# facebookresearch/robust_cvd

Hardware: NVIDIA H100
Metric: flow_residual_constraints_per_sec_per_gn_iteration (higher is better)
Workload: dtype f64

## Files before the change

robust_cvd_b200/csrc/rcvd_api.cu:

```cuda
#include <algorithm>
#include <chrono>
#include <cmath>
#include <cstdarg>
#include <cstdio>
#include <cstring>
#include <dlfcn.h>
#include <limits>
#include <map>
#include <mutex>
#include <string>
#include <vector>

#include <cub/device/device_segmented_sort.cuh>
#include "rcvd_eval.cuh"
#include "rcvd_linalg.cuh"
#include "rcvd_update.cuh"
#include "rcvd_plan.h"
#include "rcvd_cg.cuh"
#include "rcvd_selinv.cuh"
#include "rcvd_host.h"

using namespace rcvd;

static thread_local std::string g_err = "";
// ... 107 lines not shown
  if (e >= nf * nf) return;
  const int i = e / nf, j = e % nf;
  const HBlock hbk = hb[b];
  if (hbk.r == hbk.c && j > i) return;
  const double v = H[(size_t)b * npad * npad + (size_t)i * npad + j];
  const size_t U = (size_t)N * nf;
  const int ur = uperm[hbk.r], uc = uperm[hbk.c];
  out[((size_t)ur * nf + i) * U + (size_t)uc * nf + j] = v;
  out[((size_t)uc * nf + j) * U + (size_t)ur * nf + i] = v;
}

enum { LP_POTRF_SMEM = 0, LP_POTRF_PANEL, LP_TRSM_LL4, LP_TRSM_LL2, LP_TRSM_GEMM, LP_UPD_TMA1, LP_UPD_TMA2, LP_SUB_LEVEL, LP_SUB_FUSED,
       LP_TRINV, LP_OTHER, LP_UPD_TMA1_MULTI, LP_TRSM_STREAMED, LP_N };

struct RecordSet {
  const int width, nframes;
  std::vector<int32_t> frames; std::vector<int64_t> offsets{0}; std::vector<float> records;
  RecordTiles dev = {}; int num_tiles = 0;
  const float* caller_records = nullptr;
  RecordSet(int width_, int nframes_) : width(width_), nframes(nframes_) {}
  int groups() const { return (int)offsets.size() - 1; }
  int64_t count() const { return offsets.back(); }
};

struct rcvd_problem {
  rcvd_config cfg; Layout L; int N = 0; int device = 0;
  cudaStream_t stream = nullptr;
  std::vector<uint8_t> in_range; std::vector<double> median, adaptive;
  RecordSet pairs{6, 2}, trips{10, 1}, dpairs{6, 2};
  std::vector<int32_t> struct_pairs;
  int first_frame = 0, last_frame = -1;
  int32_t* d_blk_of = nullptr; uint8_t *d_in_range = nullptr, *d_active = nullptr;
  double *d_median = nullptr, *d_adaptive = nullptr; float* d_scale_locs = nullptr; int nscale = 0;
  double *d_x = nullptr, *d_xc = nullptr, *d_xsave = nullptr;
  double *d_g = nullptr, *d_S = nullptr, *d_diagH = nullptr, *d_lmdiag = nullptr, *d_D2 = nullptr, *d_gs = nullptr, *d_rhs = nullptr, *d_ytmp = nullptr,
         *d_y = nullptr, *d_Sy = nullptr, *d_Hy = nullptr, *d_partial = nullptr, *d_scal = nullptr;
  double* h_scal = nullptr;
  int part_reg = 0, part_trip = 0, part_dp = 0, npartial = 0;
  double *d_H = nullptr, *d_Lb = nullptr, *d_T = nullptr, *d_invL = nullptr, *d_invT = nullptr;
  HBlock *d_hblocks = nullptr, *d_lblocks = nullptr; int* d_fail = nullptr;
  int* d_potrf_progress = nullptr;
  FactorKernels fk = {};
  FactorPlan plan;
  int *d_lvl_frames = nullptr; TrsmTask* d_trsm_tasks = nullptr; int2* d_upd_pairs = nullptr; SolveTask* d_fwd_tasks = nullptr;
  SubTask* d_sub_tasks = nullptr; int* d_sub_counters = nullptr; int* d_sub_need = nullptr;
  cudaGraphExec_t solve_graph = nullptr;
  bool structure_ready = false;
  int nranks = 1, rank = 0; nccl::Comm comm = nullptr;
  int64_t launches = 0, graph_launches = 0;
  std::vector<double> h_state; bool state_dirty = true; bool overlap = true; int order_slack = 4;
  cudaStream_t side_stream = nullptr; cudaEvent_t ev_fork = nullptr, ev_join = nullptr;
  std::vector<cudaEvent_t> ev_side;
  cudaStream_t inv_stream = nullptr; cudaEvent_t ev_inv_join = nullptr;
  double *d_g2 = nullptr, *d_delta = nullptr; int* h_fail = nullptr;
  cudaEvent_t ev[8] = {nullptr};
  std::vector<void*> allocs;
  std::vector<std::pair<int, cudaEvent_t>>* prof = nullptr;
  bool eval_only = false;
  bool records_sorted = false;
  int fast_path = 1;
  bool dist_enabled = true, graph_warm = false, force_full_H = false;
  int *d_lvl_own = nullptr, *d_load_lblocks = nullptr, *d_own_hblocks = nullptr, *d_uperm = nullptr;
  UpdItem* d_upd_items = nullptr; CUtensorMap tmapT; int num_sms = 0, upd_ipc = 0, upd_order = 1;
  std::vector<double> level_ms;
  bool factored = false;
  int64_t paths[LP_N] = {0}, graph_paths[LP_N] = {0};
  bool use_cg = false; int64_t factor_budget = -1; uint64_t total_mem = 0;
  LinearStorage storage = {}; int64_t linear_bytes = 0;
  double cg_eta = kCgEta;
  double *d_cg_r = nullptr, *d_cg_z = nullptr, *d_cg_p = nullptr, *d_cg_q = nullptr, *d_cg_slots = nullptr, *d_cg_part = nullptr;
  int *d_cg_frames = nullptr, *d_cg_off = nullptr, *d_cg_ids = nullptr; CgState* d_cg = nullptr;
  int64_t cg_iterations = 0; int cg_max = 0, cg_capped = 0, cg_steps = 0, cg_last = 0;
  bool sel_ready = false; SelPlan sel;
  SelTile* d_sel_tiles = nullptr; SelOp* d_sel_ops = nullptr; SelTrmm* d_sel_trmm = nullptr; int *d_sel_row_off = nullptr, *d_sel_row_blk = nullptr;
  int64_t sel_launches[5] = {0}; double sel_ms[3] = {0.0, 0.0, 0.0};
  rcvd_problem() {}
};

template <class... Params, class... Args>
static int launch(rcvd_problem* p, void (*kernel)(Params...), dim3 grid, dim3 block, size_t smem, cudaStream_t s, bool pdl, Args... args) {
  if (int rc = launch_kernel(kernel, grid, block, smem, s, pdl, args...)) return rc;
  p->launches += 1;
  return RCVD_OK;
}

template <class T> static int dalloc(rcvd_problem* p, T** ptr, size_t count) {
  *ptr = nullptr;
  if (count == 0) count = 1;
  cudaError_t e = cudaMallocAsync((void**)ptr, count * sizeof(T), p->stream);
  if (e != cudaSuccess) return set_err(RCVD_ERR_CUDA, "cudaMallocAsync(%zu bytes) failed: %s", count * sizeof(T), cudaGetErrorString(e));
  p->allocs.push_back(*ptr);
  return RCVD_OK;
}
template <class T> static int upload(rcvd_problem* p, T** ptr, const std::vector<T>& v) {
  int rc = dalloc(p, ptr, v.size()); if (rc) return rc;
  if (!v.empty()) CK(cudaMemcpyAsync(*ptr, v.data(), v.size() * sizeof(T), cudaMemcpyHostToDevice, p->stream));
  return RCVD_OK;
}
template <class T> static std::vector<T> frames_to_internal(const std::vector<int>& uperm, const T* src, size_t src_stride, size_t dst_stride, size_t count, T pad = T()) {
  std::vector<T> out(uperm.size() * dst_stride, pad);
  for (size_t i = 0; i < uperm.size(); ++i) std::copy_n(src + (size_t)uperm[i] * src_stride, count, out.begin() + i * dst_stride);
  return out;
}
template <class T> static void frames_to_caller(const std::vector<int>& uperm, const T* src, size_t src_stride, T* dst, size_t dst_stride, size_t count) {
  for (size_t i = 0; i < uperm.size(); ++i) std::copy_n(src + i * src_stride, count, dst + (size_t)uperm[i] * dst_stride);
}
// ... 200 lines not shown
  if (fk.trsm_ll4) {
    CK(cudaFuncSetAttribute(k_trsm_ll<4>, cudaFuncAttributeMaxDynamicSharedMemorySize, (int)fk.trsm_ll4_bytes));
    CK(cudaFuncSetAttribute(k_trsm_ll<4, true>, cudaFuncAttributeMaxDynamicSharedMemorySize, (int)fk.trsm_ll4_bytes));
  }
  if (fk.potrf_smem) CK(cudaFuncSetAttribute(k_potrf_smem, cudaFuncAttributeMaxDynamicSharedMemorySize, (int)fk.potrf_bytes));
  return RCVD_OK;
}

static int build_structure(rcvd_problem* p) {
  if (p->nranks > 1 && !p->dpairs.frames.empty()) return set_err(RCVD_ERR_INVALID, "depth-normalisation pairs are not sharded: they need a single-GPU problem (nranks = 1)");
  free_all(p);
  CK(cudaSetDevice(p->device));
  std::vector<int32_t> graph = p->struct_pairs.empty() ? p->pairs.frames : p->struct_pairs;
  graph.insert(graph.end(), p->dpairs.frames.begin(), p->dpairs.frames.end());
  if (const char* e = make_factor_plan(p->plan, p->cfg, graph, p->trips.frames, p->order_slack, p->nranks, p->rank, p->dist_enabled, p->num_sms))
    return set_err(RCVD_ERR_INVALID, "%s", e);
  p->storage = linear_storage(p->plan, p->N, p->L.npad);
  p->use_cg = p->nranks == 1 && !p->eval_only && p->storage.cholesky > (p->factor_budget >= 0 ? p->factor_budget : cholesky_budget(p->total_mem));
  while (p->ev_side.size() < 2 * p->plan.levels.size()) { cudaEvent_t e; CK(cudaEventCreateWithFlags(&e, cudaEventDisableTiming)); p->ev_side.push_back(e); }
  int rc;
  if ((rc = upload_plan(p)) || (rc = set_up_problem_data(p)) || (rc = allocate_storage(p))) return rc;
  CK(cudaStreamSynchronize(p->stream));
  p->structure_ready = true;
  return RCVD_OK;
}

static int allreduce(rcvd_problem* p, double* buf, size_t count) {
  if (p->nranks <= 1) return RCVD_OK;
  const int r = nccl::AllReduce(buf, buf, count, nccl::kFloat64, nccl::kSum, p->comm, p->stream);
  if (r != 0) return set_err(RCVD_ERR_NCCL, "ncclAllReduce failed: %s", nccl::GetErrorString ? nccl::GetErrorString(r) : "?");
  return RCVD_OK;
}
struct Seg { size_t first, count; };
static int grouped(rcvd_problem* p, double* base, size_t unit, const std::vector<Seg>& segs, bool bcast) {
  int r = nccl::GroupStart();
  for (size_t i = 0; i < segs.size() && r == 0; ++i) {
    if (segs[i].count == 0) continue;
    const int root = (int)(i % (size_t)p->nranks);
    double* ptr = base + segs[i].first * unit;
    r = bcast ? nccl::Broadcast(ptr, ptr, segs[i].count * unit, nccl::kFloat64, root, p->comm, p->stream)
              : nccl::Reduce(ptr, ptr, segs[i].count * unit, nccl::kFloat64, nccl::kSum, root, p->comm, p->stream);
  }
  const int r2 = nccl::GroupEnd();
  if (r == 0) r = r2;
  if (r != 0) return set_err(RCVD_ERR_NCCL, "grouped NCCL %s failed: %s", bcast ? "broadcast" : "reduce", nccl::GetErrorString ? nccl::GetErrorString(r) : "?");
  return RCVD_OK;
}

struct FactorSolve {
  enum { P_LOAD = 0, P_POTRF, P_TRINV, P_TRSM, P_GEMM, P_SOLVE };
  rcvd_problem* p; const FactorPlan& pl; const FactorKernels& fk; const int N, npad, strips; cudaStream_t st, side, inv;
  int prof_level = 0;
  bool side_used = false, inv_used = false;
  int side_joined = -1;

  explicit FactorSolve(rcvd_problem* p_)
      : p(p_), pl(p_->plan), fk(p_->fk), N(p_->N), npad(p_->L.npad), strips((npad + kTrsmStrip - 1) / kTrsmStrip), st(p_->stream), side(p_->side_stream),
        inv(p_->inv_stream) {}

  void mark(int cls) {
    if (!p->prof) return;
    cudaEvent_t e; cudaEventCreate(&e); cudaEventRecord(e, st); p->prof->push_back({cls < 0 ? cls : (cls | (prof_level << 8)), e});
  }
  template <class... Params, class... Args>
  int launch(int path, void (*kernel)(Params...), dim3 grid, dim3 block, size_t smem, cudaStream_t s, bool pdl, Args... args) {
    if (int rc = ::launch(p, kernel, grid, block, smem, s, pdl, args...)) return rc;
    p->paths[path]++;
    return RCVD_OK;
  }
  int wait(cudaStream_t waiter, cudaStream_t from, cudaEvent_t e) {
    CK(cudaEventRecord(e, from)); CK(cudaStreamWaitEvent(waiter, e, 0));
    return RCVD_OK;
  }
  int join_all(int level) {
    if (side_used) { if (int rc = wait(st, side, p->ev_join)) return rc; side_joined = 2 * level - 1; }
    if (inv_used) { if (int rc = wait(st, inv, p->ev_inv_join)) return rc; inv_used = false; }
    return RCVD_OK;
  }

  bool trsm_deep(const Level& v) const { return strips * v.ntrsm <= p->num_sms && fk.trsm_ll4; }
  bool streamed(const Level& v) const {
    return fk.trsm_ll && v.nown > 0 && v.ntrsm > 0 && fk.potrf_smem && strips * v.ntrsm <= (trsm_deep(v) ? 1 : fk.trsm2_ctas_per_sm) * p->num_sms;
  }

  int factor_diagonal(const int* frames, int nfr, bool pdl) {
    if (fk.potrf_smem)
      return launch(LP_POTRF_SMEM, k_potrf_smem, dim3(nfr), dim3(kPotrfSmemThreads), fk.potrf_bytes, st, pdl, p->d_Lb, p->d_invT, frames, npad,
                    p->d_fail, p->d_potrf_progress);
    for (int jb = 0; jb < npad / 16; ++jb) {
      if (int rc = launch(LP_POTRF_PANEL, k_potrf_panel, dim3(nfr), dim3(kPotrfThreads), 0, st, false, p->d_Lb, p->d_invT, frames, npad, jb, p->d_fail)) return rc;
      const int m = npad - (jb + 1) * 16, n64 = (m + 63) / 64;
      if (m > 0) { if (int rc = launch(LP_OTHER, k_potrf_trail, dim3(n64 * (n64 + 1) / 2, nfr), dim3(128), 0, st, false, p->d_Lb, frames, npad, jb)) return rc; }
    }
    return RCVD_OK;
  }

  int trsm(const Level& lv, const int* frames, int nfr, bool chain) {
    const bool inv_stream = fk.trsm_ll && p->overlap;
    if (inv_stream) { if (int rc = wait(inv, st, p->ev_fork)) return rc; inv_used = true; }
    if (int rc = launch(LP_TRINV, k_trinv, dim3(npad / 16, nfr), dim3(256), fk.trinv_bytes, inv_stream ? inv : st, false,
                        p->d_Lb, p->d_invT, p->d_invL, frames, npad)) return rc;
    mark(P_TRINV);
    if (lv.ntrsm == 0) return RCVD_OK;
    int rc;
    if (fk.trsm_ll) {
      const bool deep = trsm_deep(lv);
      decltype(&k_trsm_ll<2>) kernel = deep ? (chain ? k_trsm_ll<4, true> : k_trsm_ll<4>) : (chain ? k_trsm_ll<2, true> : k_trsm_ll<2>);
      if (chain) p->paths[LP_TRSM_STREAMED]++;
      rc = launch(deep ? LP_TRSM_LL4 : LP_TRSM_LL2, kernel, dim3(strips, lv.ntrsm), dim3(128), deep ? fk.trsm_ll4_bytes : fk.trsm_ll2_bytes, st, chain,
                  p->d_T, p->d_Lb, p->d_invT, p->d_trsm_tasks + lv.trsm_off, npad, chain ? p->d_potrf_progress : nullptr);
    } else {
      const int tiles = (npad + 63) / 64;
      rc = launch(LP_TRSM_GEMM, k_gemm_nt, dim3(tiles, tiles, lv.ntrsm), dim3(128), 0, st, false, p->d_T, p->d_Lb, p->d_invL,
                  p->d_trsm_tasks + lv.trsm_off, npad);
    }
    if (rc) return rc;
    mark(P_TRSM);
    return RCVD_OK;
  }

  int update(cudaStream_t s, int off, int n) {
    const UpdItem* items = p->d_upd_items + (size_t)p->upd_order * pl.upd_items.size() + off;
    if (n <= p->num_sms)
      return launch(LP_UPD_TMA2, k_update_tma<2>, dim3(n), dim3(UpdShape<2>::threads), upd_smem_bytes(pl.upd_rb, 2), s, false,
                    p->tmapT, p->d_Lb, items, n, p->d_upd_pairs, npad, pl.upd_neff, pl.upd_rb, 0);
    int grid = upd_ctas(n, p->num_sms);
    if (p->upd_ipc > 0) grid = std::max(grid, (n + p->upd_ipc - 1) / p->upd_ipc);
    if (grid < n) p->paths[LP_UPD_TMA1_MULTI]++;
    return launch(LP_UPD_TMA1, k_update_tma<1>, dim3(grid), dim3(UpdShape<1>::threads), upd_smem_bytes(pl.upd_rb, 1), s, false,
                  p->tmapT, p->d_Lb, items, n, p->d_upd_pairs, npad, pl.upd_neff, pl.upd_rb, 0);
  }

  int updates(int li) {
    const Level& lv = pl.levels[li];
    const bool u2 = lv.nit2[0] + lv.nit2[1] > 0;
    const bool fork_late = li + 1 < (int)pl.levels.size() && streamed(pl.levels[li + 1]);
    if (p->overlap && u2 && !fork_late) { if (int rc = wait(side, st, p->ev_fork)) return rc; }
    if (p->overlap) {
      int s = -1;
      for (int q = side_joined + 1; q < 2 * li; ++q) { const Level& v = pl.levels[q / 2]; if (v.nit2[q % 2] > 0 && v.join[q % 2] <= li) s = q; }
      if (s >= 0) { CK(cudaStreamWaitEvent(st, p->ev_side[s], 0)); side_joined = s; }
    }
    if (lv.nit > 0) { if (int rc = update(st, lv.it_off, lv.nit)) return rc; mark(P_GEMM); }
    if (p->overlap && u2 && fork_late) { if (int rc = wait(side, st, p->ev_fork)) return rc; }
    for (int h = 0; h < 2; ++h) if (lv.nit2[h] > 0) {
      if (int rc = update(p->overlap ? side : st, lv.it2_off[h], lv.nit2[h])) return rc;
      mark(P_GEMM);
      if (p->overlap) { CK(cudaEventRecord(p->ev_side[2 * li + h], side)); side_used = true; }
    }
    return RCVD_OK;
  }

  int broadcast_level(int li) {
    std::vector<Seg> segs;
    for (int q = 0; q < p->nranks; ++q) segs.push_back({(size_t)pl.tseg[(li * p->nranks + q) * 2], (size_t)pl.tseg[(li * p->nranks + q) * 2 + 1]});
    return grouped(p, p->d_T, (size_t)npad * npad, segs, true);
  }
  int phase_boundary() {
    if (int rc = join_all(pl.LB)) return rc;
    const size_t bsz = (size_t)npad * npad;
    std::vector<Seg> invs, tr;
    for (int q = 0; q < p->nranks; ++q) invs.push_back({(size_t)pl.fa_off[q], (size_t)pl.fa_cnt[q]});
    for (int q = 0; q < p->nranks; ++q) tr.push_back({(size_t)pl.fb_off[q], (size_t)pl.fb_cnt[q]});
    for (int q = 0; q < p->nranks; ++q) tr.push_back({(size_t)N + (size_t)pl.bseg[2 * q], (size_t)pl.bseg[2 * q + 1]});
    if (int rc = grouped(p, p->d_invL, bsz, invs, true)) return rc;
    return grouped(p, p->d_Lb, bsz, tr, true);
  }

  int substitution() {
    CK(cudaMemcpyAsync(p->d_rhs, p->d_gs, (size_t)N * npad * sizeof(double), cudaMemcpyDeviceToDevice, st));
    const int LS = pl.sub_first_level;
    int rc;
    for (int l = 0; l < LS; ++l) {
      const Level& lv = pl.levels[l];
      if ((rc = launch(LP_SUB_LEVEL, k_fwd_diag, dim3((npad + 7) / 8, lv.nframes), dim3(256), 0, st, false, p->d_invL, p->d_rhs, p->d_ytmp,
                       p->d_lvl_frames + lv.frame_off, npad, nullptr))) return rc;
      if (lv.nfwd > 0 && (rc = launch(LP_SUB_LEVEL, k_fwd_update, dim3((npad + 7) / 8, lv.nfwd), dim3(256), 0, st, false, p->d_T, p->d_ytmp, p->d_rhs,
                                      p->d_fwd_tasks + lv.fwd_off, npad))) return rc;
    }
    if (LS < (int)pl.levels.size() && !pl.sub_tasks.empty()) {
      CK(cudaMemsetAsync(p->d_sub_counters, 0, ((size_t)4 * N + 4) * sizeof(int), st));
      SubCounters cn; cn.ticket = p->d_sub_counters; cn.fin = p->d_sub_counters + 4; cn.fdone = cn.fin + N; cn.bin = cn.fdone + N; cn.bdone = cn.bin + N;
      cn.fin_need = p->d_sub_need; cn.bin_need = p->d_sub_need + N;
      const int ntasks = (int)pl.sub_tasks.size();
      if ((rc = launch(LP_SUB_FUSED, k_substitution, dim3(std::min(ntasks, p->num_sms)), dim3(kSubThreads), fk.substitution_bytes, st, false,
                       p->d_invL, p->d_T, p->d_rhs, p->d_ytmp, p->d_y, p->d_sub_tasks, ntasks, cn, npad))) return rc;
    }
    for (int l = LS - 1; l >= 0; --l) {
      const Level& lv = pl.levels[l];
      if (lv.nfwd > 0 && (rc = launch(LP_SUB_LEVEL, k_bwd_update, dim3((npad + 31) / 32, lv.nfwd), dim3(256), 0, st, false, p->d_T, p->d_y, p->d_ytmp,
                                      p->d_fwd_tasks + lv.fwd_off, npad))) return rc;
      if ((rc = launch(LP_SUB_LEVEL, k_bwd_diag, dim3((npad + 31) / 32, lv.nframes), dim3(256), 0, st, false, p->d_invL, p->d_ytmp, p->d_y,
                       p->d_lvl_frames + lv.frame_off, npad, nullptr))) return rc;
    }
    mark(P_SOLVE);
    return RCVD_OK;
  }
};

static int enqueue_factor_solve(rcvd_problem* p) {
  FactorSolve f(p);
  const FactorPlan& pl = p->plan; const int npad = p->L.npad, nlv = (int)pl.levels.size();
  f.mark(-1);
  CK(cudaMemsetAsync(p->d_potrf_progress, 0, (size_t)p->N * sizeof(int), p->stream));
  const int nfill = (int)pl.load_lblocks.size() - pl.nload;
  if (int rc = f.launch(LP_OTHER, k_load_factor, dim3((npad * npad + 255) / 256, pl.nload + load_factor_pad_rows(npad, pl.upd_neff, nfill)), dim3(256), 0,
                        p->stream, false, p->d_H, p->d_Lb, p->d_lblocks, p->d_S, p->d_D2, npad, p->L.nf, pl.upd_neff, p->d_load_lblocks, pl.nload, nfill)) return rc;
  f.mark(FactorSolve::P_LOAD);
  for (int li = 0; li < nlv; ++li) {
    const Level& lv = pl.levels[li]; f.prof_level = li;
    if (pl.dist && li == pl.LB) { if (int rc = f.phase_boundary()) return rc; }
    if (lv.nown > 0) {
      const int* frames = p->d_lvl_own + lv.own_off;
      const bool chain = f.streamed(lv);
      if (int rc = f.factor_diagonal(frames, lv.nown, chain && li > 0)) return rc;
      f.mark(FactorSolve::P_POTRF);
      if (int rc = f.trsm(lv, frames, lv.nown, chain)) return rc;
    }
    if (pl.dist && li < pl.LB) { if (int rc = f.broadcast_level(li)) return rc; }
    if (int rc = f.updates(li)) return rc;
  }
  if (pl.dist && pl.LB >= nlv) { if (int rc = f.phase_boundary()) return rc; }
  if (int rc = f.join_all(nlv)) return rc;
  if (int rc = f.substitution()) return rc;
  CK(cudaGetLastError());
  return RCVD_OK;
}

static int factor_solve(rcvd_problem* p) {
  if (p->nranks > 1 && !p->graph_warm) {
    p->graph_warm = true; p->factored = true;
    return enqueue_factor_solve(p);
  }
  if (!p->solve_graph) {
    cudaGraph_t graph;
    const int64_t l0 = p->launches;
    int64_t paths0[LP_N]; std::copy(p->paths, p->paths + LP_N, paths0);
    CK(cudaStreamBeginCapture(p->stream, cudaStreamCaptureModeThreadLocal));
    int rc = enqueue_factor_solve(p);
    cudaError_t e = cudaStreamEndCapture(p->stream, &graph);
    for (int i = 0; i < LP_N; ++i) { p->graph_paths[i] = p->paths[i] - paths0[i]; p->paths[i] = paths0[i]; }
    if (rc) return rc;
    if (e != cudaSuccess) return set_err(RCVD_ERR_CUDA, "graph capture failed: %s", cudaGetErrorString(e));
    CK(cudaGraphInstantiate(&p->solve_graph, graph, 0));
    cudaGraphDestroy(graph);
    p->graph_launches = p->launches - l0;
    p->launches = l0;
  }
  CK(cudaGraphLaunch(p->solve_graph, p->stream));
  p->launches += p->graph_launches;
  for (int i = 0; i < LP_N; ++i) p->paths[i] += p->graph_paths[i];
  p->factored = true;
  return RCVD_OK;
}

static int enqueue_cg_preconditioner(rcvd_problem* p) {
  FactorSolve f(p);
  const int N = p->N, npad = p->L.npad;
  if (int rc = f.launch(LP_OTHER, k_load_factor, dim3((npad * npad + 255) / 256, N), dim3(256), 0, p->stream, false, p->d_H, p->d_Lb, p->d_lblocks,
                        p->d_S, p->d_D2, npad, p->L.nf, p->plan.upd_neff, p->d_cg_frames, N, 0)) return rc;
  if (int rc = f.factor_diagonal(p->d_cg_frames, N, false)) return rc;
  return f.launch(LP_TRINV, k_trinv, dim3(npad / 16, N), dim3(256), p->fk.trinv_bytes, p->stream, false, p->d_Lb, p->d_invT, p->d_invL, p->d_cg_frames, npad);
}

static int enqueue_cg_product(rcvd_problem* p, const double* v, double* out, const CgState* cg) {
  const int N = p->N, npad = p->L.npad, nf = p->L.nf, nH = (int)p->plan.hblocks.size();
  const size_t smem = (size_t)(3 * npad + 8 * 256) * sizeof(double);
  if (int rc = launch(p, k_cg_spmv, nH, kCgThreads, smem, p->stream, false, p->d_H, p->d_hblocks, p->d_S, v, p->d_cg_slots, nH, npad, nf, cg)) return rc;
  return launch(p, k_cg_gather, N, kCgThreads, 0, p->stream, false, p->d_cg_slots, p->d_cg_off, p->d_cg_ids, p->d_S, p->d_D2, v, out, p->d_cg_part, npad, nf, cg);
}

static int enqueue_cg_iteration(rcvd_problem* p, int i) {
  const int N = p->N, npad = p->L.npad, n = N * npad;
  cudaStream_t st = p->stream; const int* stop = &p->d_cg->stop; double* x = p->d_y; int rc;
  auto apply = [&](const double* v, double* out) { return enqueue_cg_product(p, v, out, p->d_cg); };
  auto scalar = [&](int phase, int nparts) {
    return launch(p, k_cg_scalar, 1, kCgThreads, 0, st, false, p->d_cg_part, nparts, p->d_cg, p->d_fail, phase, p->cg_eta, kCgMaxIterations);
  };
  auto step = [&](int mode) {
    return launch(p, k_cg_step, kCgDotBlocks, kCgThreads, 0, st, false, x, p->d_cg_p, p->d_cg_r, p->d_cg_q, p->d_gs, p->d_cg_part, n, mode, p->d_cg);
  };
  if ((rc = launch(p, k_fwd_diag, dim3((npad + 7) / 8, N), 256, 0, st, false, p->d_invL, p->d_cg_r, p->d_ytmp, p->d_cg_frames, npad, stop)) ||
      (rc = launch(p, k_bwd_diag, dim3((npad + 31) / 32, N), 256, 0, st, false, p->d_invL, p->d_ytmp, p->d_cg_z, p->d_cg_frames, npad, stop)) ||
      (rc = launch(p, k_cg_dot, kCgDotBlocks, kCgThreads, 0, st, false, p->d_cg_r, p->d_cg_z, p->d_cg_part, n, p->d_cg)) || (rc = scalar(CG_RHO, kCgDotBlocks)) ||
      (rc = launch(p, k_cg_direction, kCgDotBlocks, kCgThreads, 0, st, false, p->d_cg_z, p->d_cg_p, n, p->d_cg)))
    return rc;
  if ((rc = apply(p->d_cg_p, p->d_cg_q)) || (rc = scalar(CG_CURVATURE, N))) return rc;
  if (i % kCgResetPeriod != 0) rc = step(0);
  else if (!(rc = step(1)) && !(rc = apply(x, p->d_cg_q))) rc = step(2);
  return rc ? rc : scalar(CG_MODEL, kCgDotBlocks);
}

static int cg_solve(rcvd_problem* p) {
  cudaStream_t st = p->stream; int rc;
  if ((rc = enqueue_cg_preconditioner(p)) ||
      (rc = launch(p, k_cg_init, kCgDotBlocks, kCgThreads, 0, st, false, p->d_gs, p->d_y, p->d_cg_r, p->d_cg_part, p->N * p->L.npad)) ||
      (rc = launch(p, k_cg_scalar, 1, kCgThreads, 0, st, false, p->d_cg_part, kCgDotBlocks, p->d_cg, p->d_fail, (int)CG_INIT, p->cg_eta, kCgMaxIterations)))
    return rc;
  CgState h;
  for (int i = 1;; ) {
    for (int k = 0; k < kCgChunk && i <= kCgMaxIterations; ++k, ++i) if ((rc = enqueue_cg_iteration(p, i))) return rc;
    CK(cudaMemcpyAsync(&h, p->d_cg, sizeof(h), cudaMemcpyDeviceToHost, st));
    CK(cudaStreamSynchronize(st));
    if (h.stop || i > kCgMaxIterations) break;
  }
  p->cg_last = h.iterations; p->cg_iterations += h.iterations; p->cg_max = std::max(p->cg_max, h.iterations);
  p->cg_capped += h.capped; p->cg_steps += 1;
  return RCVD_OK;
}

static int linear_solve(rcvd_problem* p) { return p->use_cg ? cg_solve(p) : factor_solve(p); }


static int enqueue_evaluate(rcvd_problem* p, const double* x, bool wantG, bool wantH, double* gout, int slot) {
  if (wantH && p->eval_only) return set_err(RCVD_ERR_INVALID, "this handle was set to evaluation-only (rcvd_debug_set_eval_only): no normal matrix");
// ... 282 lines not shown
  CK(cudaStreamSynchronize(st));
  sum.iterations = iter; sum.final_cost = minimumCost;
  sum.gpu_launches = p->launches - launches0;
  sum.total_ms = std::chrono::duration<double, std::milli>(clk::now() - t0).count();
  return RCVD_OK;
}

RCVD_API const char* rcvd_last_error(void) { return g_err.c_str(); }
RCVD_API int32_t rcvd_abi_version(void) { return 1; }
RCVD_API int32_t rcvd_frame_stride(const rcvd_config* c) { Layout L; return (c && make_layout(*c, L)) ? L.nf : -1; }
RCVD_API int32_t rcvd_depth_param_offset(const rcvd_config* c) { Layout L; return (c && make_layout(*c, L)) ? L.offD : -1; }
RCVD_API int32_t rcvd_spatial_param_offset(const rcvd_config* c) { Layout L; return (c && make_layout(*c, L)) ? L.offS : -1; }
RCVD_API void rcvd_default_solve_options(rcvd_solve_options* o) {
  o->max_iterations = 1000; o->verbose = 0; o->function_tolerance = 1e-6; o->gradient_tolerance = 1e-10; o->parameter_tolerance = 1e-8;
  o->initial_radius = 1e4; o->max_radius = 1e16; o->min_radius = 1e-32; o->min_relative_decrease = 1e-3; o->min_lm_diagonal = 1e-6;
  o->max_lm_diagonal = 1e32; o->max_consecutive_invalid_steps = 5; o->jacobi_scaling = 1;
}

static cudaError_t device_total_mem(int device, uint64_t* out) {
  static std::mutex m; static std::map<int, uint64_t> cache;
  std::lock_guard<std::mutex> lock(m);
  auto it = cache.find(device);
  if (it == cache.end()) {
    cudaDeviceProp prop;
    if (cudaError_t e = cudaGetDeviceProperties(&prop, device)) return e;
    it = cache.emplace(device, (uint64_t)prop.totalGlobalMem).first;
  }
  *out = it->second;
  return cudaSuccess;
}
RCVD_API int32_t rcvd_problem_create(const rcvd_config* cfg, int32_t device, rcvd_problem** out) {
  if (!cfg || !out) return set_err(RCVD_ERR_INVALID, "null argument");
  Layout L;
  if (!make_layout(*cfg, L) || cfg->num_frames <= 0) return set_err(RCVD_ERR_INVALID, "unsupported transform configuration");
  if (int rc = check_device(device)) return rc;
  SET_DEVICE(device);
  {
    cudaMemPool_t pool; unsigned long long keep = ~0ull;
    if (cudaDeviceGetDefaultMemPool(&pool, device) == cudaSuccess) cudaMemPoolSetAttribute(pool, cudaMemPoolAttrReleaseThreshold, &keep);
  }
  rcvd_problem* p = new rcvd_problem();
  p->cfg = *cfg; p->L = L; p->N = cfg->num_frames; p->device = device;
  p->in_range.assign(p->N, 1); p->median.assign(p->N, 1.0); p->h_state.assign((size_t)p->N * L.nf, 0.0);
  cudaError_t e = cudaDeviceGetAttribute(&p->num_sms, cudaDevAttrMultiProcessorCount, device);
  if (e == cudaSuccess) e = device_total_mem(device, &p->total_mem);
  if (e != cudaSuccess) { delete p; return set_err(RCVD_ERR_CUDA, "cudaDeviceGetAttribute / cudaGetDeviceProperties: %s", cudaGetErrorString(e)); }
  int prio_lo = 0, prio_hi = 0; cudaDeviceGetStreamPriorityRange(&prio_lo, &prio_hi);
  e = cudaStreamCreateWithPriority(&p->stream, cudaStreamNonBlocking, prio_hi);
  if (e == cudaSuccess) e = cudaStreamCreateWithPriority(&p->side_stream, cudaStreamNonBlocking, prio_lo);
  if (e == cudaSuccess) e = cudaStreamCreateWithPriority(&p->inv_stream, cudaStreamNonBlocking, prio_lo);
  if (e == cudaSuccess) e = cudaEventCreateWithFlags(&p->ev_fork, cudaEventDisableTiming);
  if (e == cudaSuccess) e = cudaEventCreateWithFlags(&p->ev_join, cudaEventDisableTiming);
  if (e == cudaSuccess) e = cudaEventCreateWithFlags(&p->ev_inv_join, cudaEventDisableTiming);
  for (int i = 0; i < 8 && e == cudaSuccess; ++i) e = cudaEventCreate(&p->ev[i]);
  if (e != cudaSuccess) { rcvd_problem_destroy(p); return set_err(RCVD_ERR_CUDA, "cudaStreamCreate / cudaEventCreate: %s", cudaGetErrorString(e)); }
  *out = p; return RCVD_OK;
}
RCVD_API void rcvd_problem_destroy(rcvd_problem* p) {
  if (!p) return;
  DevGuard dev_guard_(p->device);
  free_all(p);
  for (int i = 0; i < 8; ++i) if (p->ev[i]) cudaEventDestroy(p->ev[i]);
  if (p->comm && nccl::CommDestroy) nccl::CommDestroy(p->comm);
  if (p->ev_fork) cudaEventDestroy(p->ev_fork);
  if (p->ev_join) cudaEventDestroy(p->ev_join);
  for (cudaEvent_t e : p->ev_side) cudaEventDestroy(e);
  if (p->ev_inv_join) cudaEventDestroy(p->ev_inv_join);
  if (p->side_stream) cudaStreamDestroy(p->side_stream);
  if (p->inv_stream) cudaStreamDestroy(p->inv_stream);
  if (p->stream) cudaStreamDestroy(p->stream);
  delete p;
}
RCVD_API int32_t rcvd_problem_set_frames(rcvd_problem* p, const uint8_t* in_range, const double* median, const double* adaptive) {
  if (!p) return set_err(RCVD_ERR_INVALID, "null problem");
  const bool grid = adaptive && p->cfg.depth_type == RCVD_DEPTH_GRID;
  if (p->cfg.adaptive_deform > 0.0 && !grid) return set_err(RCVD_ERR_INVALID, "adaptive deformation cost requires node weights");
  if (int rc = drop_structure(p)) return rc;
  if (in_range) p->in_range.assign(in_range, in_range + p->N); else p->in_range.assign(p->N, 1);
  if (median) p->median.assign(median, median + p->N); else p->median.assign(p->N, 1.0);
  if (grid) p->adaptive.assign(adaptive, adaptive + (size_t)p->N * p->cfg.depth_grid_x * p->cfg.depth_grid_y); else p->adaptive.clear();
  return RCVD_OK;
}
static int32_t set_records(rcvd_problem* p, RecordSet rcvd_problem::*family, const char* what, int32_t n, const int32_t* frames, const int64_t* off,
                           const float* rec) {
  if (!p || n < 0 || (n > 0 && (!frames || !off))) return set_err(RCVD_ERR_INVALID, "bad %s arrays", what);
  RecordSet& s = p->*family;
  if (n > 0 && off[0] != 0) return set_err(RCVD_ERR_INVALID, "%s offsets must start at 0", what);
  for (int i = 0; i < n; ++i) {
    if (off[i + 1] < off[i]) return set_err(RCVD_ERR_INVALID, "%s offsets must be non-decreasing", what);
    const int32_t* f = frames + (size_t)i * s.nframes;
    const bool ok = s.nframes == 2 ? f[0] >= 0 && f[0] < p->N && f[1] >= 0 && f[1] < p->N && f[0] != f[1]
                                   : f[0] >= 1 && f[0] < p->N - 1;
    if (!ok) return set_err(RCVD_ERR_INVALID, "bad %s group %d", what, i);
  }
  const int64_t count = n > 0 ? off[n] : 0;
  if (count > 0 && !rec) return set_err(RCVD_ERR_INVALID, "null %s records", what);
  if (int rc = drop_structure(p)) return rc;
  s.frames.assign(frames, frames + (size_t)n * s.nframes);
  if (n > 0) s.offsets.assign(off, off + n + 1); else s.offsets.assign(1, 0);
  s.records.assign(rec, rec + (size_t)count * s.width);
  return RCVD_OK;
}
RCVD_API int32_t rcvd_problem_set_constraints(rcvd_problem* p, int32_t np, const int32_t* pf, const int64_t* off, const float* rec) {
  return set_records(p, &rcvd_problem::pairs, "constraint", np, pf, off, rec);
}
RCVD_API int32_t rcvd_problem_set_triplets(rcvd_problem* p, int32_t nt, const int32_t* centers, const int64_t* off, const float* rec) {
  return set_records(p, &rcvd_problem::trips, "triplet", nt, centers, off, rec);
}
RCVD_API int32_t rcvd_problem_set_depth_pairs(rcvd_problem* p, int32_t np, const int32_t* pf, const int64_t* off, const float* rec) {
  if (p && p->nranks > 1 && np > 0) return set_err(RCVD_ERR_INVALID, "depth-normalisation pairs are not sharded: they need a single-GPU problem (nranks = 1)");
  return set_records(p, &rcvd_problem::dpairs, "depth-pair", np, pf, off, rec);
}
RCVD_API int32_t rcvd_problem_set_structure(rcvd_problem* p, int32_t np, const int32_t* pf) {
  if (!p || np < 0 || (np > 0 && !pf)) return set_err(RCVD_ERR_INVALID, "bad structure arrays");
  if (int rc = drop_structure(p)) return rc;
  p->struct_pairs.assign(pf, pf + 2 * (size_t)np);
  return RCVD_OK;
}
RCVD_API int32_t rcvd_nccl_unique_id(uint8_t out[128]) {
  if (!nccl::load()) return set_err(RCVD_ERR_NCCL, "libnccl.so.2 not found");
// ... 761 lines not shown
```

robust_cvd_b200/csrc/rcvd_linalg.cuh:

```cuda
#pragma once
#include "rcvd_device.cuh"
#include "rcvd_ptx.cuh"

namespace rcvd {

constexpr int kPotrfThreads = 256;

__global__ void __launch_bounds__(kPotrfThreads) k_potrf_panel(double* __restrict__ Lb, double* __restrict__ invT,
                                                                const int* __restrict__ frames, int npad, int jb, int* __restrict__ fail) {
  __shared__ double D[16][17];
  __shared__ double Di[16][17];
  const int frame = frames[blockIdx.x];
  double* A = Lb + (size_t)frame * npad * npad;
  double* iT = invT + (size_t)frame * npad * 16;
  const int tid = threadIdx.x;
  const int j0 = jb * 16;
  {
    const int r = tid >> 4, cc = tid & 15;
    D[r][cc] = (cc <= r) ? A[(size_t)(j0 + r) * npad + j0 + cc] : 0.0;
  }
  __syncthreads();
  if (tid < 32) {
    const int i = tid;
    for (int j = 0; j < 16; ++j) {
// ... 218 lines not shown
      const int cidx = lane;
      double xcol[16];
#pragma unroll
      for (int r = 0; r < 16; ++r) xcol[r] = (r == cidx) ? 1.0 : 0.0;
#pragma unroll
      for (int q = 0; q < 16; q += 2) {
        const double2 pq = *reinterpret_cast<const double2*>(&pv[q]);
        const double2 dq = *reinterpret_cast<const double2*>(&D[swz(q + 1, q)]);
        xcol[q] *= pq.x;
        xcol[q + 1] = (xcol[q + 1] - xcol[q] * dq.x) * pq.y;
#pragma unroll
        for (int r = 0; r < 16; ++r) if (r > q + 1) { const double2 l = *reinterpret_cast<const double2*>(&D[swz(r, q)]); xcol[r] -= l.x * xcol[q]; xcol[r] -= l.y * xcol[q + 1]; }
      }
#pragma unroll
      for (int r = 0; r < 16; ++r) iT[(size_t)jb * 256 + r * 16 + cidx] = xcol[r];
    }
    POTRF_PHASE(2);
    if (warp != 0) named_bar_sync<3, kPotrfSmemThreads - 32>();
    POTRF_PHASE(3);
    const int m = nt - jb - 1, ntr = m * (m + 1) / 2;
    auto upd_tile = [&](int gi, int gj) -> double* {
      const double* Xi = tiles + (size_t)(gi * (gi + 1) / 2 + jb) * kTileSz;
      const double* Xj = tiles + (size_t)(gj * (gj + 1) / 2 + jb) * kTileSz;
      double* Ct = tiles + (size_t)(gi * (gi + 1) / 2 + gj) * kTileSz;
      double acc[2][2][2] = {{{0.0, 0.0}, {0.0, 0.0}}, {{0.0, 0.0}, {0.0, 0.0}}};
      tile_mma_nt(Xi, Xj, acc, g, t);
#pragma unroll
      for (int i = 0; i < 2; ++i)
#pragma unroll
        for (int j = 0; j < 2; ++j) {
          double2* ptr = reinterpret_cast<double2*>(&Ct[swz(i * 8 + g, j * 8 + 2 * t)]);
          double2 v = *ptr; v.x -= acc[i][j][0]; v.y -= acc[i][j][1]; *ptr = v;
        }
      return Ct;
    };
    if (warp == 0) {
      double* Ct = nullptr;
      if (ntr > 0) { __syncwarp(); Ct = upd_tile(jb + 1, jb + 1); }
      __threadfence_block();
      named_bar_arrive<2, kPotrfSmemThreads>();
      POTRF_PHASE(4);
      if (ntr > 0) { __syncwarp(); warp_chol16_blocked(Ct, pinv + (jb + 1) * 16, lane, fail); }
      POTRF_PHASE(5);
    } else {
      for (int tl = 1 + widx; tl < ntr; tl += nwork) { const int2 tij = tri_index(tl); upd_tile(jb + 1 + tij.x, jb + 1 + tij.y); }
    }
    POTRF_PHASE(6);
    __syncthreads();
    POTRF_PHASE(7);
  }
  if (warp != 0) publish(nt - 1);
}

__global__ void __launch_bounds__(256) k_trinv(const double* __restrict__ Lb, const double* __restrict__ invT, double* __restrict__ invL,
                                                const int* __restrict__ frames, int npad) {
  extern __shared__ double Z[];
  __shared__ double W[16][17];
  const int frame = frames[blockIdx.y];
  const int j = blockIdx.x;
  const int nt = npad / 16;
  double* Lrow_s = Z + (size_t)nt * 256;
  const int ldp = npad + 1;
  const double* A = Lb + (size_t)frame * npad * npad;
  const double* iT = invT + (size_t)frame * npad * 16;
  double* out = invL + (size_t)frame * npad * npad;
  const int tid = threadIdx.x, r = tid >> 4, c = tid & 15;
  for (int i = 0; i < j; ++i) out[(size_t)(i * 16 + r) * npad + j * 16 + c] = 0.0;
  Z[(size_t)j * 256 + tid] = iT[(size_t)j * 256 + tid];
  out[(size_t)(j * 16 + r) * npad + j * 16 + c] = Z[(size_t)j * 256 + tid];
  __syncthreads();
  for (int i = j + 1; i < nt; ++i) {
    const int kw = (i - j) * 16;
    for (int e = tid; e < 16 * kw; e += 256) { const int rr = e / kw, kk = e % kw; Lrow_s[rr * ldp + kk] = A[(size_t)(i * 16 + rr) * npad + j * 16 + kk]; }
    __syncthreads();
    double s0 = 0.0, s1 = 0.0, s2 = 0.0, s3 = 0.0;
    const double* lr = Lrow_s + r * ldp;
    const double* zp = Z + (size_t)j * 256 + c;
    for (int kk = 0; kk < kw; kk += 4) {
      s0 += lr[kk] * zp[(size_t)kk * 16]; s1 += lr[kk + 1] * zp[(size_t)(kk + 1) * 16];
      s2 += lr[kk + 2] * zp[(size_t)(kk + 2) * 16]; s3 += lr[kk + 3] * zp[(size_t)(kk + 3) * 16];
    }
    W[r][c] = (s0 + s1) + (s2 + s3);
    __syncthreads();
    double zv = 0.0;
    const double* ti = iT + (size_t)i * 256;
#pragma unroll
    for (int q = 0; q < 16; ++q) zv -= ti[r * 16 + q] * W[q][c];
    Z[(size_t)i * 256 + tid] = zv;
    out[(size_t)(i * 16 + r) * npad + j * 16 + c] = zv;
    __syncthreads();
  }
}

struct TrsmTask { int dst; int src; int kframe; };

constexpr int kGemmLd = 20;

template <int NI, int NJ>
__device__ __forceinline__ void gemm_stage(const double* __restrict__ as, const double* __restrict__ bsm, double (&acc)[4][4][2], int wm, int wn, int g, int t) {
#pragma unroll
  for (int k4 = 0; k4 < 4; ++k4) {
    double af[NI > 0 ? NI : 1], bf[NJ > 0 ? NJ : 1];
#pragma unroll
    for (int i = 0; i < NI; ++i) af[i] = as[(wm + i * 8 + g) * kGemmLd + k4 * 4 + t];
#pragma unroll
    for (int j = 0; j < NJ; ++j) bf[j] = bsm[(wn + j * 8 + g) * kGemmLd + k4 * 4 + t];
#pragma unroll
    for (int i = 0; i < NI; ++i)
#pragma unroll
      for (int j = 0; j < NJ; ++j) dmma_8x8x4(acc[i][j][0], acc[i][j][1], af[i], bf[j]);
  }
}

__global__ void __launch_bounds__(128, 4) k_gemm_nt(double* __restrict__ T, const double* __restrict__ Lb, const double* __restrict__ invL,
                                                  const TrsmTask* __restrict__ tasks, int npad) {
  __shared__ __align__(16) double As[2][64 * kGemmLd];
  __shared__ __align__(16) double Bs[2][64 * kGemmLd];
  const TrsmTask task = tasks[blockIdx.z];
  const int m0 = blockIdx.y * 64, n0 = blockIdx.x * 64;
  const size_t bs = (size_t)npad * npad;
  const int tid = threadIdx.x, warp = tid >> 5, lane = tid & 31;
  const int wm = (warp >> 1) * 32, wn = (warp & 1) * 32;
  const int g = lane >> 2, t = lane & 3;
  const int kchunks = min(npad, n0 + 64) / 16;
  const int ni = min(4, max(0, (npad - (m0 + wm)) / 8)), nj = min(4, max(0, (npad - (n0 + wn)) / 8));
  double acc[4][4][2];
#pragma unroll
  for (int i = 0; i < 4; ++i)
#pragma unroll
    for (int j = 0; j < 4; ++j) { acc[i][j][0] = 0.0; acc[i][j][1] = 0.0; }

  auto load_stage = [&](int st, int kk) {
    const double* Ag = Lb + (size_t)task.src * bs + kk * 16;
    const double* Bg = invL + (size_t)task.kframe * bs + kk * 16;
#pragma unroll
    for (int q = 0; q < 4; ++q) {
      const int cidx = tid + q * 128;
      const int row = cidx >> 3, kc = (cidx & 7) * 2;
      const bool va = (m0 + row) < npad, vb = (n0 + row) < npad;
      cp_async16(&As[st][row * kGemmLd + kc], Ag + (size_t)(va ? m0 + row : 0) * npad + kc, va);
      cp_async16(&Bs[st][row * kGemmLd + kc], Bg + (size_t)(vb ? n0 + row : 0) * npad + kc, vb);
    }
    cp_async_commit();
  };
// ... 328 lines not shown
            const int row = r0 + i;
            const int len = tk.type == 0 ? row + 1 : npad;
            m[qi][i] = (row < c1 && q < len) ? *reinterpret_cast<const double2*>(M + (size_t)row * npad + q) : make_double2(0.0, 0.0);
            if (q + 1 >= len) m[qi][i].y = 0.0;
          }
        }
        if (qb == 0) dep_wait();
        double2 v[4];
#pragma unroll
        for (int qi = 0; qi < 4; ++qi) { const int q = qb + qi * 64 + 2 * lane; v[qi] = q < npad ? ldcg2(vin + q) : make_double2(0.0, 0.0); }
#pragma unroll
        for (int qi = 0; qi < 4; ++qi)
#pragma unroll
          for (int i = 0; i < RW; ++i) acc[i] += m[qi][i].x * v[qi].x + m[qi][i].y * v[qi].y;
      }
#pragma unroll
      for (int i = 0; i < RW; ++i) {
        const double sum = warp_sum(acc[i]);
        const int row = r0 + i;
        if (lane == 0 && row < c1) { if (tk.type == 0) y[(size_t)tk.k * npad + row] = sum; else red_add(rhs + (size_t)tk.r * npad + row, -sum); }
      }
    } else {
      const int cl = tid & 31, rg = tid >> 5, j = c0 + 2 * cl;
      double ax = 0.0, ay = 0.0;
      const int ifirst = tk.type == 3 ? j + ((rg - j) & 7) : rg;
      for (int ib = ifirst; ib < npad || ib == ifirst; ib += 256) {
        double2 m[32];
#pragma unroll
        for (int u = 0; u < 32; ++u) { const int i = ib + 8 * u; m[u] = (i < npad && j < c1) ? *reinterpret_cast<const double2*>(M + (size_t)i * npad + j) : make_double2(0.0, 0.0); }
        if (ib == ifirst) dep_wait();
        double vi[32];
#pragma unroll
        for (int u = 0; u < 32; ++u) { const int i = ib + 8 * u; vi[u] = i < npad ? __ldcg(vin + i) : 0.0; }
#pragma unroll
        for (int u = 0; u < 32; ++u) { const int i = ib + 8 * u; ax += m[u].x * vi[u]; if (tk.type != 3 || i > j) ay += m[u].y * vi[u]; }
      }
      red[rg * (kSubChunk + 2) + 2 * cl] = ax; red[rg * (kSubChunk + 2) + 2 * cl + 1] = ay;
      __syncthreads();
      if (tid < kSubChunk && c0 + tid < c1) {
        double sum = 0.0;
#pragma unroll
        for (int q = 0; q < 8; ++q) sum += red[q * (kSubChunk + 2) + tid];
        if (tk.type == 3) x[(size_t)tk.k * npad + c0 + tid] = sum; else red_add(y + (size_t)tk.k * npad + c0 + tid, -sum);
      }
    }
    __syncthreads();
    if (tid == 0) red_release_add(tk.type == 0 ? cn.fdone + tk.k : (tk.type == 1 ? cn.fin + tk.r : (tk.type == 2 ? cn.bin + tk.k : cn.bdone + tk.k)), 1);
  }
}

struct FactorKernels {
  bool potrf_smem, trsm_ll, trsm_ll4;
  size_t potrf_bytes, trsm_ll2_bytes, trsm_ll4_bytes, trinv_bytes, substitution_bytes;
  int trsm2_ctas_per_sm;
};
inline FactorKernels factor_kernels(int npad) {
  const size_t potrf = potrf_smem_bytes(npad), ll2 = trsm_ll_smem_bytes(npad, 2), ll4 = trsm_ll_smem_bytes(npad, 4);
  const size_t trinv = (size_t)(npad * 16 + 16 * (npad + 1)) * sizeof(double);
  const size_t sub = (size_t)8 * (kSubChunk + 2) * sizeof(double);
  return {potrf <= kMaxDynSmem, ll2 <= kMaxDynSmem, ll4 <= kMaxDynSmem, potrf, ll2, ll4, trinv, sub, 0};
}

struct HBlock { int lblk; int r; int c; };
__global__ void __launch_bounds__(256) k_load_factor(const double* __restrict__ H, double* __restrict__ Lb, const HBlock* __restrict__ lb,
                                                      const double* __restrict__ S, const double* __restrict__ D2, int npad, int nf, int neff,
                                                      const int* __restrict__ blist, int nload, int nfill) {
  const size_t bs = (size_t)npad * npad;
  if ((int)blockIdx.y >= nload) {
    const int ph = npad - neff, per = ph * (npad + neff);
    const long q = ((long)(blockIdx.y - nload) * gridDim.x + blockIdx.x) * 256 + threadIdx.x;
    if (per == 0 || q >= (long)nfill * per) return;
    const int f = (int)(q / per), e = (int)(q % per), r = e - ph * npad;
    const int i = r < 0 ? neff + e / npad : r / ph, j = r < 0 ? e % npad : neff + r % ph;
    Lb[(size_t)blist[nload + f] * bs + (size_t)i * npad + j] = 0.0;
    return;
  }
  const int bid = blist[blockIdx.y];
  const HBlock b = lb[bid];
  const int e = blockIdx.x * 256 + threadIdx.x;
  if (e >= npad * npad) return;
  const int i = e / npad, j = e % npad;
  double v = 0.0;
  if (b.r == b.c) {
    if (j > i) v = 0.0;
    else if (i >= nf) v = (i == j) ? 1.0 : 0.0;
    else {
      v = H[(size_t)b.lblk * bs + e] * S[(size_t)b.r * npad + i] * S[(size_t)b.c * npad + j];
      if (i == j) v += D2[(size_t)b.r * npad + i];
    }
  } else if (i < nf && j < nf) {
    v = H[(size_t)b.lblk * bs + e] * S[(size_t)b.r * npad + i] * S[(size_t)b.c * npad + j];
  }
  Lb[(size_t)bid * bs + e] = v;
}
__host__ __device__ inline int load_factor_pad_rows(int npad, int neff, int nfill) {
  const long per = (long)(npad - neff) * (npad + neff), row = (long)((npad * npad + 255) / 256) * 256;
  return (int)(((long)nfill * per + row - 1) / row);
}

__global__ void __launch_bounds__(256) k_spmv_sym(const double* __restrict__ H, const HBlock* __restrict__ hb, const double* __restrict__ v,
                                                   double* __restrict__ out, int npad, const int* __restrict__ blist) {
  const int bid = blist ? blist[blockIdx.y] : blockIdx.y;
  const HBlock b = hb[bid];
  const int row = blockIdx.x * 8 + (threadIdx.x >> 5);
  const int lane = threadIdx.x & 31;
  if (row >= npad) return;
  const double* M = H + (size_t)bid * npad * npad + (size_t)row * npad;
  const double* vc = v + (size_t)b.c * npad;
  const double vr = v[(size_t)b.r * npad + row];
  double s = 0.0;
  if (b.r == b.c) {
    for (int q = lane; q <= row; q += 32) {
      const double m = M[q];
// ... 16 lines not shown
```

Before: 87.89 million.

## Double-buffer trinv row loads with cp.async and start substitution before final inverse join

k_trinv now stages each L row block and its diagonal inverse into shared memory with cp.async, prefetching the next block while the current one is computed, so global load latency is hidden. Separately, the forward substitution no longer waits for the whole inverse stream. It waits on an event recorded after the last trinv needed by the dense substitution levels, and joins the inverse stream fully only before the sub-task phase. The cost is more shared memory per block, which may lower occupancy, and more complex stream dependencies.

```diff
diff --git a/robust_cvd_b200/csrc/rcvd_api.cu b/robust_cvd_b200/csrc/rcvd_api.cu
--- a/robust_cvd_b200/csrc/rcvd_api.cu
+++ b/robust_cvd_b200/csrc/rcvd_api.cu
@@ -183,6 +183,7 @@
   cudaStream_t side_stream = nullptr; cudaEvent_t ev_fork = nullptr, ev_join = nullptr;
   std::vector<cudaEvent_t> ev_side;
   cudaStream_t inv_stream = nullptr; cudaEvent_t ev_inv_join = nullptr;
+  cudaEvent_t ev_inv_wide = nullptr;
   double *d_g2 = nullptr, *d_delta = nullptr; int* h_fail = nullptr;
   cudaEvent_t ev[8] = {nullptr};
   std::vector<void*> allocs;
@@ -489,6 +490,7 @@
   rcvd_problem* p; const FactorPlan& pl; const FactorKernels& fk; const int N, npad, strips; cudaStream_t st, side, inv;
   int prof_level = 0;
   bool side_used = false, inv_used = false;
+  bool inv_wide = false;
   int side_joined = -1;
 
   explicit FactorSolve(rcvd_problem* p_)
@@ -509,9 +511,9 @@
     CK(cudaEventRecord(e, from)); CK(cudaStreamWaitEvent(waiter, e, 0));
     return RCVD_OK;
   }
-  int join_all(int level) {
+  int join_all(int level, bool with_inv = true) {
     if (side_used) { if (int rc = wait(st, side, p->ev_join)) return rc; side_joined = 2 * level - 1; }
-    if (inv_used) { if (int rc = wait(st, inv, p->ev_inv_join)) return rc; inv_used = false; }
+    if (with_inv && inv_used) { if (int rc = wait(st, inv, p->ev_inv_join)) return rc; inv_used = false; inv_wide = false; }
     return RCVD_OK;
   }
 
@@ -536,7 +538,8 @@
     const bool inv_stream = fk.trsm_ll && p->overlap;
     if (inv_stream) { if (int rc = wait(inv, st, p->ev_fork)) return rc; inv_used = true; }
     if (int rc = launch(LP_TRINV, k_trinv, dim3(npad / 16, nfr), dim3(256), fk.trinv_bytes, inv_stream ? inv : st, false,
-                        p->d_Lb, p->d_invT, p->d_invL, frames, npad)) return rc;
+                        p->d_Lb, p->d_invT, p->d_invL, frames, npad, fk.trinv_ahead)) return rc;
+    if (inv_stream && &lv - pl.levels.data() == pl.sub_first_level - 1) { CK(cudaEventRecord(p->ev_inv_wide, inv)); inv_wide = true; }
     mark(P_TRINV);
     if (lv.ntrsm == 0) return RCVD_OK;
     int rc;
@@ -608,6 +611,8 @@
     CK(cudaMemcpyAsync(p->d_rhs, p->d_gs, (size_t)N * npad * sizeof(double), cudaMemcpyDeviceToDevice, st));
     const int LS = pl.sub_first_level;
     int rc;
+    if (inv_wide) { CK(cudaStreamWaitEvent(st, p->ev_inv_wide, 0)); inv_wide = false; }
+    else if (inv_used) { if ((rc = wait(st, inv, p->ev_inv_join))) return rc; inv_used = false; }
     for (int l = 0; l < LS; ++l) {
       const Level& lv = pl.levels[l];
       if ((rc = launch(LP_SUB_LEVEL, k_fwd_diag, dim3((npad + 7) / 8, lv.nframes), dim3(256), 0, st, false, p->d_invL, p->d_rhs, p->d_ytmp,
@@ -615,6 +620,7 @@
       if (lv.nfwd > 0 && (rc = launch(LP_SUB_LEVEL, k_fwd_update, dim3((npad + 7) / 8, lv.nfwd), dim3(256), 0, st, false, p->d_T, p->d_ytmp, p->d_rhs,
                                       p->d_fwd_tasks + lv.fwd_off, npad))) return rc;
     }
+    if (inv_used) { if ((rc = wait(st, inv, p->ev_inv_join))) return rc; inv_used = false; }
     if (LS < (int)pl.levels.size() && !pl.sub_tasks.empty()) {
       CK(cudaMemsetAsync(p->d_sub_counters, 0, ((size_t)4 * N + 4) * sizeof(int), st));
       SubCounters cn; cn.ticket = p->d_sub_counters; cn.fin = p->d_sub_counters + 4; cn.fdone = cn.fin + N; cn.bin = cn.fdone + N; cn.bdone = cn.bin + N;
@@ -658,7 +664,7 @@
     if (int rc = f.updates(li)) return rc;
   }
   if (pl.dist && pl.LB >= nlv) { if (int rc = f.phase_boundary()) return rc; }
-  if (int rc = f.join_all(nlv)) return rc;
+  if (int rc = f.join_all(nlv, false)) return rc;
   if (int rc = f.substitution()) return rc;
   CK(cudaGetLastError());
   return RCVD_OK;
@@ -697,7 +703,8 @@
   if (int rc = f.launch(LP_OTHER, k_load_factor, dim3((npad * npad + 255) / 256, N), dim3(256), 0, p->stream, false, p->d_H, p->d_Lb, p->d_lblocks,
                         p->d_S, p->d_D2, npad, p->L.nf, p->plan.upd_neff, p->d_cg_frames, N, 0)) return rc;
   if (int rc = f.factor_diagonal(p->d_cg_frames, N, false)) return rc;
-  return f.launch(LP_TRINV, k_trinv, dim3(npad / 16, N), dim3(256), p->fk.trinv_bytes, p->stream, false, p->d_Lb, p->d_invT, p->d_invL, p->d_cg_frames, npad);
+  return f.launch(LP_TRINV, k_trinv, dim3(npad / 16, N), dim3(256), p->fk.trinv_bytes, p->stream, false, p->d_Lb, p->d_invT, p->d_invL, p->d_cg_frames, npad,
+                  p->fk.trinv_ahead);
 }
 
 static int enqueue_cg_product(rcvd_problem* p, const double* v, double* out, const CgState* cg) {
@@ -1086,6 +1093,7 @@
   if (e == cudaSuccess) e = cudaEventCreateWithFlags(&p->ev_fork, cudaEventDisableTiming);
   if (e == cudaSuccess) e = cudaEventCreateWithFlags(&p->ev_join, cudaEventDisableTiming);
   if (e == cudaSuccess) e = cudaEventCreateWithFlags(&p->ev_inv_join, cudaEventDisableTiming);
+  if (e == cudaSuccess) e = cudaEventCreateWithFlags(&p->ev_inv_wide, cudaEventDisableTiming);
   for (int i = 0; i < 8 && e == cudaSuccess; ++i) e = cudaEventCreate(&p->ev[i]);
   if (e != cudaSuccess) { rcvd_problem_destroy(p); return set_err(RCVD_ERR_CUDA, "cudaStreamCreate / cudaEventCreate: %s", cudaGetErrorString(e)); }
   *out = p; return RCVD_OK;
@@ -1100,6 +1108,7 @@
   if (p->ev_join) cudaEventDestroy(p->ev_join);
   for (cudaEvent_t e : p->ev_side) cudaEventDestroy(e);
   if (p->ev_inv_join) cudaEventDestroy(p->ev_inv_join);
+  if (p->ev_inv_wide) cudaEventDestroy(p->ev_inv_wide);
   if (p->side_stream) cudaStreamDestroy(p->side_stream);
   if (p->inv_stream) cudaStreamDestroy(p->inv_stream);
   if (p->stream) cudaStreamDestroy(p->stream);
diff --git a/robust_cvd_b200/csrc/rcvd_linalg.cuh b/robust_cvd_b200/csrc/rcvd_linalg.cuh
--- a/robust_cvd_b200/csrc/rcvd_linalg.cuh
+++ b/robust_cvd_b200/csrc/rcvd_linalg.cuh
@@ -294,29 +294,42 @@
   if (warp != 0) publish(nt - 1);
 }
 
+__host__ __device__ inline size_t trinv_slot_doubles(int npad) { return (size_t)16 * (npad + 2) + 256; }
+__host__ __device__ inline size_t trinv_smem_bytes(int npad, int ahead) { return ((size_t)npad * 16 + ahead * trinv_slot_doubles(npad)) * sizeof(double); }
+
 __global__ void __launch_bounds__(256) k_trinv(const double* __restrict__ Lb, const double* __restrict__ invT, double* __restrict__ invL,
-                                                const int* __restrict__ frames, int npad) {
-  extern __shared__ double Z[];
+                                                const int* __restrict__ frames, int npad, int ahead) {
+  extern __shared__ __align__(16) double Z[];
   __shared__ double W[16][17];
   const int frame = frames[blockIdx.y];
   const int j = blockIdx.x;
   const int nt = npad / 16;
-  double* Lrow_s = Z + (size_t)nt * 256;
-  const int ldp = npad + 1;
+  const int ld = npad + 2;
+  double* slots = Z + (size_t)nt * 256;
   const double* A = Lb + (size_t)frame * npad * npad;
   const double* iT = invT + (size_t)frame * npad * 16;
   double* out = invL + (size_t)frame * npad * npad;
   const int tid = threadIdx.x, r = tid >> 4, c = tid & 15;
+  auto stage = [&](int i) {
+    if (i < nt) {
+      double* ls = slots + (size_t)((i - j - 1) % ahead) * trinv_slot_doubles(npad);
+      const int w = (i - j) * 8;
+      for (int e = tid; e < 16 * w; e += 256) { const int rr = e / w, kc = (e - rr * w) * 2; cp_async16(&ls[rr * ld + kc], A + (size_t)(i * 16 + rr) * npad + j * 16 + kc); }
+      if (tid < 128) cp_async16(&ls[16 * ld + tid * 2], iT + (size_t)i * 256 + tid * 2);
+    }
+    cp_async_commit();
+  };
+  if (ahead > 1) stage(j + 1);
   for (int i = 0; i < j; ++i) out[(size_t)(i * 16 + r) * npad + j * 16 + c] = 0.0;
   Z[(size_t)j * 256 + tid] = iT[(size_t)j * 256 + tid];
   out[(size_t)(j * 16 + r) * npad + j * 16 + c] = Z[(size_t)j * 256 + tid];
-  __syncthreads();
   for (int i = j + 1; i < nt; ++i) {
+    if (ahead > 1) { stage(i + 1); cp_async_wait<1>(); } else { stage(i); cp_async_wait<0>(); }
+    __syncthreads();
+    const double* ls = slots + (size_t)((i - j - 1) % ahead) * trinv_slot_doubles(npad);
     const int kw = (i - j) * 16;
-    for (int e = tid; e < 16 * kw; e += 256) { const int rr = e / kw, kk = e % kw; Lrow_s[rr * ldp + kk] = A[(size_t)(i * 16 + rr) * npad + j * 16 + kk]; }
-    __syncthreads();
     double s0 = 0.0, s1 = 0.0, s2 = 0.0, s3 = 0.0;
-    const double* lr = Lrow_s + r * ldp;
+    const double* lr = ls + r * ld;
     const double* zp = Z + (size_t)j * 256 + c;
     for (int kk = 0; kk < kw; kk += 4) {
       s0 += lr[kk] * zp[(size_t)kk * 16]; s1 += lr[kk + 1] * zp[(size_t)(kk + 1) * 16];
@@ -325,13 +338,14 @@
     W[r][c] = (s0 + s1) + (s2 + s3);
     __syncthreads();
     double zv = 0.0;
-    const double* ti = iT + (size_t)i * 256;
+    const double* ti = ls + 16 * ld;
 #pragma unroll
     for (int q = 0; q < 16; ++q) zv -= ti[r * 16 + q] * W[q][c];
     Z[(size_t)i * 256 + tid] = zv;
     out[(size_t)(i * 16 + r) * npad + j * 16 + c] = zv;
     __syncthreads();
   }
+  cp_async_wait<0>();
 }
 
 struct TrsmTask { int dst; int src; int kframe; };
@@ -766,13 +780,14 @@
 struct FactorKernels {
   bool potrf_smem, trsm_ll, trsm_ll4;
   size_t potrf_bytes, trsm_ll2_bytes, trsm_ll4_bytes, trinv_bytes, substitution_bytes;
+  int trinv_ahead;
   int trsm2_ctas_per_sm;
 };
 inline FactorKernels factor_kernels(int npad) {
   const size_t potrf = potrf_smem_bytes(npad), ll2 = trsm_ll_smem_bytes(npad, 2), ll4 = trsm_ll_smem_bytes(npad, 4);
-  const size_t trinv = (size_t)(npad * 16 + 16 * (npad + 1)) * sizeof(double);
+  const int trinv_ahead = trinv_smem_bytes(npad, 2) <= kMaxDynSmem ? 2 : 1;
   const size_t sub = (size_t)8 * (kSubChunk + 2) * sizeof(double);
-  return {potrf <= kMaxDynSmem, ll2 <= kMaxDynSmem, ll4 <= kMaxDynSmem, potrf, ll2, ll4, trinv, sub, 0};
+  return {potrf <= kMaxDynSmem, ll2 <= kMaxDynSmem, ll4 <= kMaxDynSmem, potrf, ll2, ll4, trinv_smem_bytes(npad, trinv_ahead), sub, trinv_ahead, 0};
 }
 
 struct HBlock { int lblk; int r; int c; };
```

After: 88.80 million (median of 6 runs). +1.0%, better.
